# BharathMasetty/DPG-SLAM

Measured on AMD Instinct MI355X. Metric: ICP edges/sec + ms/GN-iter on 5k-node/20k-edge synthetic graph, 1->8 GPU, higher is better.
Workload: dtype fp32 (ICP) + fp64 (GN)

## Files before the change

### dpg-slam_amd/csrc/dpg_chol.h

```cpp
#ifndef DPG_CHOL_H
#define DPG_CHOL_H

#include <stdint.h>

#include <vector>

struct dpg_chol_opts {
    int32_t max_supernode_cols = 64;
    double relax_fraction = 0.3;
    int32_t order = 0;
    int32_t merge_single = 0;
    int32_t fused = 1;
    int32_t solve_stage = -1;
    int32_t solve_maxseg = -1;
    int32_t solve_dinv = 0;
    int32_t solve_inv_cols = 0;
};

struct dpg_chol_sym {
    int64_t n = 0;
    int32_t ns = 0;
    int32_t n_levels = 0;
    int32_t max_front = 0;
    double flops = 0.0;
    std::vector<int32_t> perm, pos;
    std::vector<int32_t> sn_c0;
    std::vector<int32_t> sn_of;
    std::vector<int64_t> sn_rows_ptr;
    std::vector<int32_t> sn_rows;
    std::vector<int32_t> sn_parent;
    std::vector<int32_t> sn_level;
    std::vector<int32_t> level_ptr;
    std::vector<int32_t> level_list;
    std::vector<int64_t> child_ptr;
    std::vector<int32_t> child_list;
    std::vector<int32_t> relmap;
    std::vector<int64_t> front_off;
};

int dpg_chol_symbolic(int64_t n, const int32_t* pair_lo, const int32_t* pair_hi, int64_t n_pairs,
                      const dpg_chol_opts* opts, dpg_chol_sym* S);
int dpg_chol_order(int64_t n, const int32_t* pair_lo, const int32_t* pair_hi, int64_t n_pairs,
                   std::vector<int32_t>& perm, std::vector<std::vector<int32_t>>& pat, bool md = false);
int dpg_chol_order_nd(int64_t n, const int32_t* pair_lo, const int32_t* pair_hi, int64_t n_pairs, int32_t leaf,
                      std::vector<int32_t>& perm, std::vector<std::vector<int32_t>>& pat);
int dpg_chol_order_nd_sep(int64_t n, const int32_t* pair_lo, const int32_t* pair_hi, int64_t n_pairs, int32_t leaf,
                          int32_t starts, int32_t bal, int32_t score, bool cover, std::vector<int32_t>& perm,
                          std::vector<std::vector<int32_t>>& pat, bool par = false);
int dpg_chol_sym_from_patterns(int64_t n, const std::vector<int32_t>& perm, const std::vector<std::vector<int32_t>>& pat,
                               const dpg_chol_opts* opts, dpg_chol_sym* S);
double dpg_chol_critical_path_us(const dpg_chol_sym& S);
int dpg_chol_sym_from_csr(int64_t n, const int32_t* perm, const int64_t* cp, const int32_t* prow,
                          const dpg_chol_opts* opts, dpg_chol_sym* S);

struct dpg_chol_incsym {
    int64_t n = 0, words = 0;
    std::vector<int32_t> perm, pos;
    std::vector<uint64_t> bits;
    int64_t swords = 0;
    std::vector<uint64_t> summ;
    std::vector<int32_t> parent;
    int64_t nnz = 0;
    std::vector<int64_t> cp;
    std::vector<int32_t> rows, rows_tmp;
    std::vector<std::pair<int32_t, int32_t>> added;
};
int dpg_incsym_reset(dpg_chol_incsym* I, int64_t n, const int32_t* pair_lo, const int32_t* pair_hi, int64_t n_pairs,
                     const dpg_chol_opts* opts = nullptr);
int dpg_incsym_order(int64_t n, const int32_t* pair_lo, const int32_t* pair_hi, int64_t n_pairs,
                     std::vector<int32_t>& perm, std::vector<std::vector<int32_t>>& pat,
                     const dpg_chol_opts* opts = nullptr, bool concurrent = false);
void dpg_incsym_init(dpg_chol_incsym* I, int64_t n, std::vector<int32_t>& perm, std::vector<std::vector<int32_t>>& pat);
void dpg_incsym_append(dpg_chol_incsym* I, int64_t k);
int64_t dpg_incsym_add_edge(dpg_chol_incsym* I, int32_t a, int32_t b);
int dpg_incsym_derive(dpg_chol_incsym* I, const dpg_chol_opts* opts, dpg_chol_sym* S);


int dpg_chol_create_sym(void** h, int64_t n, const int32_t* pair_lo, const int32_t* pair_hi, int64_t n_pairs,
                        dpg_chol_sym* S, const dpg_chol_opts* opts = nullptr);
int dpg_chol_create_sym_plan(void** h, int64_t n, const int32_t* pair_lo, const int32_t* pair_hi, int64_t n_pairs,
                             dpg_chol_sym* S, const dpg_chol_opts* opts = nullptr);
int dpg_chol_create_sym_upload(void** h);
int dpg_chol_plan_blocks(void** h, int64_t n, const int32_t* pos, const int32_t* perm, const int32_t* pair_lo,
                         const int32_t* pair_hi, int64_t n_pairs);
void dpg_chol_blocks_invalidate(void* h);
void dpg_chol_build_times(void* h, double out[2]);
int dpg_chol_fused(void* h);
int dpg_chol_plan_host(int64_t n, const int32_t* pair_lo, const int32_t* pair_hi, int64_t n_pairs,
                       const dpg_chol_sym* S, const dpg_chol_opts* opts, double* ms);

#endif
```

### dpg-slam_amd/csrc/dpg_chol_sym.cpp

```cpp
#include <math.h>
#include <stdint.h>
#include <stdio.h>
#include <stdlib.h>
#include <string.h>
#include <time.h>

#include <algorithm>
#include <atomic>
#include <functional>
#include <future>
#include <memory>
#include <queue>
#include <vector>

#include "dpg_chol.h"
#include "dpg_chol_plan.h"

namespace {

void min_degree(int64_t n, const std::vector<int64_t>& aptr, const std::vector<int32_t>& adj,
                std::vector<int32_t>& perm, std::vector<std::vector<int32_t>>& pattern) {
    const int64_t W = (n + 63) / 64;
    std::vector<uint64_t> bits((size_t)(n * W), 0ull);
    std::vector<int32_t> wlo((size_t)n, (int32_t)W), whi((size_t)n, 0);
    for (int64_t v = 0; v < n; ++v)
        for (int64_t q = aptr[v]; q < aptr[v + 1]; ++q) {
            const int32_t u = adj[(size_t)q];
            bits[(size_t)(v * W + u / 64)] |= 1ull << (u % 64);
            wlo[(size_t)v] = std::min(wlo[(size_t)v], u / 64);
            whi[(size_t)v] = std::max(whi[(size_t)v], u / 64 + 1);
        }
    std::vector<int32_t> deg((size_t)n);
    for (int64_t v = 0; v < n; ++v) deg[(size_t)v] = (int32_t)(aptr[v + 1] - aptr[v]);
    std::vector<char> done((size_t)n, 0);
    perm.assign((size_t)n, -1);
    pattern.assign((size_t)n, {});
    std::vector<int32_t> nb;
    nb.reserve(1024);
    std::priority_queue<std::pair<int32_t, int32_t>, std::vector<std::pair<int32_t, int32_t>>,
                        std::greater<std::pair<int32_t, int32_t>>> heap;
    for (int64_t v = 0; v < n; ++v) heap.emplace(deg[(size_t)v], (int32_t)v);
    for (int64_t p = 0; p < n; ++p) {
        int32_t v = -1;
        while (!heap.empty()) {
            const auto top = heap.top();
            heap.pop();
            if (!done[(size_t)top.second] && top.first == deg[(size_t)top.second]) { v = top.second; break; }
        }
        done[(size_t)v] = 1;
        perm[(size_t)p] = v;
        nb.clear();
        uint64_t* bv = &bits[(size_t)(v * W)];
        const int32_t vlo = wlo[(size_t)v], vhi = whi[(size_t)v];
        for (int64_t w = vlo; w < vhi; ++w) {
            uint64_t b = bv[w];
            while (b) {
                const int t = __builtin_ctzll(b);
                b &= b - 1;
                nb.push_back((int32_t)(w * 64 + t));
            }
        }
        pattern[(size_t)p] = nb;
        for (int32_t u : nb) {
            uint64_t* bu = &bits[(size_t)(u * W)];
            for (int64_t w = vlo; w < vhi; ++w) bu[w] |= bv[w];
            bu[u / 64] &= ~(1ull << (u % 64));
            bu[v / 64] &= ~(1ull << (v % 64));
            int32_t lo = std::min(wlo[(size_t)u], vlo), hi = std::max(whi[(size_t)u], vhi);
            while (lo < hi && bu[lo] == 0) ++lo;
            while (hi > lo && bu[hi - 1] == 0) --hi;
            wlo[(size_t)u] = lo;
            whi[(size_t)u] = hi;
            int32_t d = 0;
            for (int64_t w = lo; w < hi; ++w) d += __builtin_popcountll(bu[w]);
            if (d != deg[(size_t)u]) heap.emplace(d, u);
            deg[(size_t)u] = d;
        }
        for (int64_t w = vlo; w < vhi; ++w) bv[w] = 0;
    }
}

struct NdParams {
    int32_t starts = 0, bal = 5, score = 0;
    bool cover = false;
    bool par = false;
};
struct NdShared {
    std::vector<int32_t> stamp, lvl, aux;
    std::vector<int64_t> fptr;
    std::vector<int32_t> fcnt;
    std::atomic<int32_t> next_id{0};
};
struct NdState {
    int64_t n;
    const int64_t* aptr;
    const int32_t* adj;
    const int32_t* fadj = nullptr;
    int32_t leaf;
    NdParams prm;
    NdShared* sh;
    std::vector<int32_t> queue;
    std::vector<int32_t>* out;
};
inline int32_t stamp_of(const NdState& st, int32_t v) { return __atomic_load_n(&st.sh->stamp[(size_t)v], __ATOMIC_RELAXED); }
inline void stamp_set(NdState& st, int32_t v, int32_t id) { __atomic_store_n(&st.sh->stamp[(size_t)v], id, __ATOMIC_RELAXED); }
inline int32_t nd_new_id(NdState& st) { return st.sh->next_id.fetch_add(1, std::memory_order_relaxed) + 1; }

inline const int32_t* nbr_begin(const NdState& st, int32_t v) { return st.fadj + st.sh->fptr[(size_t)v]; }
inline const int32_t* nbr_end(const NdState& st, int32_t v) { return st.fadj + st.sh->fptr[(size_t)v] + st.sh->fcnt[(size_t)v]; }

void nd_filter(NdState& st, const std::vector<int32_t>& sub, int32_t id, std::vector<int32_t>& fadj) {
    size_t tot = 0;
    for (int32_t v : sub) tot += (size_t)(st.aptr[v + 1] - st.aptr[v]);
    fadj.clear();
    fadj.reserve(tot);
    for (int32_t v : sub) {
        st.sh->fptr[(size_t)v] = (int64_t)fadj.size();
        for (int64_t t = st.aptr[v]; t < st.aptr[v + 1]; ++t) {
            const int32_t u = st.adj[(size_t)t];
            if (stamp_of(st, u) == id) fadj.push_back(u);
        }
        st.sh->fcnt[(size_t)v] = (int32_t)((int64_t)fadj.size() - st.sh->fptr[(size_t)v]);
    }
    st.fadj = fadj.data();
}

int32_t nd_bfs_into(const NdState& st, int32_t id, int32_t src, int32_t* lvl, std::vector<int32_t>& queue) {
    (void)id;
    if (queue.size() < (size_t)st.n + 1) queue.resize((size_t)st.n + 1);
    int32_t* q = queue.data();
    size_t qh = 0, qt = 1;
    q[0] = src;
    lvl[src] = 0;
    int32_t h = 0;
    while (qh < qt) {
        const int32_t v = q[qh++];
        const int32_t lv = lvl[v];
        h = std::max(h, lv);
        for (const int32_t *p = nbr_begin(st, v), *e = nbr_end(st, v); p != e; ++p) {
            const int32_t u = *p;
            const int32_t lu = lvl[u];
            const bool fresh = lu < 0;
            lvl[u] = fresh ? lv + 1 : lu;
            q[qt] = u;
            qt += fresh;
        }
    }
    queue.resize(qt);
    return h + 1;
}
int32_t nd_bfs(NdState& st, int32_t id, int32_t src) { return nd_bfs_into(st, id, src, st.sh->lvl.data(), st.queue); }

int32_t nd_degree(const NdState& st, int32_t id, int32_t v) {
    (void)id;
    return st.sh->fcnt[(size_t)v];
}

void min_degree_small(int32_t n, uint64_t* row, int32_t* perm) {
    int32_t deg[64];
    uint64_t left = n == 64 ? ~0ull : ((1ull << n) - 1);
    for (int32_t v = 0; v < n; ++v) deg[v] = __builtin_popcountll(row[v]);
    for (int32_t p = 0; p < n; ++p) {
        int32_t v = -1;
        for (uint64_t m = left; m; m &= m - 1) {
            const int32_t u = __builtin_ctzll(m);
            if (v < 0 || deg[u] < deg[v]) v = u;
        }
        left &= ~(1ull << v);
        perm[p] = v;
        const uint64_t bv = row[v];
        for (uint64_t m = bv; m; m &= m - 1) {
            const int32_t u = __builtin_ctzll(m);
            row[u] = (row[u] | bv) & ~(1ull << u) & ~(1ull << v);
            deg[u] = __builtin_popcountll(row[u]);
        }
        row[v] = 0;
    }
}

void nd_min_degree(NdState& st, const std::vector<int32_t>& sub) {
    const int32_t id = nd_new_id(st);
    for (size_t i = 0; i < sub.size(); ++i) { stamp_set(st, sub[i], id); st.sh->lvl[(size_t)sub[i]] = (int32_t)i; }
    if (sub.size() <= 64) {
        uint64_t row[64];
        int32_t lp[64];
        const int32_t n = (int32_t)sub.size();
        for (int32_t i = 0; i < n; ++i) {
            const int32_t v = sub[(size_t)i];
            row[i] = 0;
            for (int64_t t = st.aptr[v]; t < st.aptr[v + 1]; ++t)
                if (stamp_of(st, st.adj[(size_t)t]) == id) row[i] |= 1ull << st.sh->lvl[(size_t)st.adj[(size_t)t]];
        }
        min_degree_small(n, row, lp);
        for (int32_t k = 0; k < n; ++k) st.out->push_back(sub[(size_t)lp[k]]);
        return;
    }
    std::vector<int64_t> ap(sub.size() + 1, 0);
    std::vector<int32_t> aj;
    for (size_t i = 0; i < sub.size(); ++i) {
        const int32_t v = sub[i];
        for (int64_t t = st.aptr[v]; t < st.aptr[v + 1]; ++t)
            if (stamp_of(st, st.adj[(size_t)t]) == id) aj.push_back(st.sh->lvl[(size_t)st.adj[(size_t)t]]);
        ap[i + 1] = (int64_t)aj.size();
    }
    std::vector<int32_t> lp;
    std::vector<std::vector<int32_t>> lpat;
    min_degree((int64_t)sub.size(), ap, aj, lp, lpat);
    for (int32_t l : lp) st.out->push_back(sub[(size_t)l]);
}

void nd_rec(NdState& st, std::vector<int32_t>& sub);

constexpr size_t kNdParMin = 1024;
void nd_halves(NdState& st, std::vector<int32_t>& A, std::vector<int32_t>& B, const std::vector<int32_t>& S) {
    if (st.prm.par && A.size() + B.size() >= kNdParMin) {
        std::vector<int32_t> outB;
        NdState sb;
        sb.n = st.n;
        sb.aptr = st.aptr;
        sb.adj = st.adj;
        sb.leaf = st.leaf;
        sb.prm = st.prm;
        sb.sh = st.sh;
        sb.out = &outB;
        std::future<void> fb = std::async(std::launch::async, [&sb, &B] { nd_rec(sb, B); });
        nd_rec(st, A);
        fb.get();
        st.out->insert(st.out->end(), outB.begin(), outB.end());
    } else {
        nd_rec(st, A);
        nd_rec(st, B);
    }
    for (int32_t v : S) st.out->push_back(v);
}

struct NdCut {
    int32_t bm = -1;
    bool up = false;
    double sc = 0.0;
    int64_t imb = 0;
};
constexpr size_t kNdStartsParMin = 2048;
constexpr size_t kNdStartsThreads = 4;
NdCut nd_best_cut(const NdState& st, const std::vector<int32_t>& sub, int32_t id, int32_t s0, int32_t* lvl,
                  std::vector<int32_t>& queue, int32_t have_h = 0) {
    NdCut best;
    const int64_t N = (int64_t)sub.size();
    int32_t hh = have_h;
    if (hh <= 0) {
        for (int32_t v : sub) lvl[v] = -1;
        hh = nd_bfs_into(st, id, s0, lvl, queue);
    }
    if (hh < 3) return best;
    std::vector<int64_t> cnt((size_t)hh, 0), slo((size_t)hh, 0), shi((size_t)hh, 0);
    for (int32_t v : sub) {
        const int32_t l = lvl[v];
        cnt[(size_t)l]++;
        bool up = false, dn = false;
        for (const int32_t *p = nbr_begin(st, v), *e = nbr_end(st, v); p != e; ++p) {
            const int32_t lu = lvl[*p];
            up |= lu == l + 1;
            dn |= lu == l - 1;
        }
        slo[(size_t)l] += up;
        if (l > 0) shi[(size_t)l - 1] += dn;
    }
    int64_t below = 0;
    for (int32_t l = 0; l + 1 < hh; ++l) {
        const bool up = shi[(size_t)l] < slo[(size_t)l];
        const int64_t sz = up ? shi[(size_t)l] : slo[(size_t)l];
        const int64_t a_sz = below + cnt[(size_t)l] - (up ? 0 : sz), b_sz = N - a_sz - sz;
        below += cnt[(size_t)l];
        if (l == 0 || (int64_t)st.prm.bal * a_sz < N || (int64_t)st.prm.bal * b_sz < N) continue;
        const double mn = (double)std::min(a_sz, b_sz);
        const double sc = st.prm.score == 2 ? (double)sz * sqrt((double)N / mn)
                          : st.prm.score == 1 ? (double)sz * (double)N / mn : (double)sz;
        const int64_t imb = a_sz > b_sz ? a_sz - b_sz : b_sz - a_sz;
        if (best.bm < 0 || sc < best.sc || (sc == best.sc && imb < best.imb)) {
            best.bm = l; best.up = up; best.sc = sc; best.imb = imb;
        }
    }
    return best;
}

void nd_split_multi(NdState& st, std::vector<int32_t>& sub, int32_t id, int32_t src, int32_t have_h) {
    const int64_t N = (int64_t)sub.size();
    const int T = N >= 256 ? st.prm.starts : 1;
    std::vector<int32_t> starts{src};
    int32_t h_src = have_h;
    {
        if (h_src <= 0) {
            for (int32_t v : sub) st.sh->lvl[(size_t)v] = -1;
            h_src = nd_bfs(st, id, src);
        }
        const std::vector<int32_t> order(st.queue.begin(), st.queue.end());
        for (int t = 1; t < T; ++t) starts.push_back(order[(size_t)((int64_t)t * (N - 1) / T)]);
        starts.push_back(order.back());
    }
    std::vector<NdCut> cuts(starts.size());
    const int W = st.prm.par && (size_t)N >= kNdStartsParMin ? (int)std::min<size_t>(kNdStartsThreads, starts.size()) : 1;
    size_t k_shared = 0;
    for (size_t k = 0; k < starts.size(); k += (size_t)W) {
        cuts[k] = nd_best_cut(st, sub, id, starts[k], st.sh->lvl.data(), st.queue, k == 0 ? h_src : 0);
        k_shared = k;
        if (k == 0 && W > 1) {
            break;
        }
    }
    if (W > 1) {
        auto work = [&](int w) {
            std::unique_ptr<int32_t[]> lv(new int32_t[(size_t)st.n]);
            std::vector<int32_t> q;
            for (size_t k = (size_t)w; k < starts.size(); k += (size_t)W) cuts[k] = nd_best_cut(st, sub, id, starts[k], lv.get(), q);
        };
        std::vector<std::future<void>> fs;
        for (int w = 1; w < W; ++w) fs.push_back(std::async(std::launch::async, work, w));
        for (size_t k = (size_t)W; k < starts.size(); k += (size_t)W) {
            cuts[k] = nd_best_cut(st, sub, id, starts[k], st.sh->lvl.data(), st.queue);
            k_shared = k;
        }
        for (auto& f : fs) f.get();
    }
    int32_t bsrc = -1, bm = -1;
    bool bupper = false;
    double bsc = 0.0;
    int64_t bimb = 0;
    for (size_t k = 0; k < starts.size(); ++k) {
        const NdCut& c = cuts[k];
        if (c.bm >= 0 && (bm < 0 || c.sc < bsc || (c.sc == bsc && c.imb < bimb))) {
            bsrc = starts[k]; bm = c.bm; bupper = c.up; bsc = c.sc; bimb = c.imb;
        }
    }
    if (bm < 0) { nd_min_degree(st, sub); return; }
    if (bsrc != starts[k_shared]) {
        for (int32_t v : sub) st.sh->lvl[(size_t)v] = -1;
        nd_bfs(st, id, bsrc);
    }
    auto touches = [&](int32_t v, int32_t l) {
        for (const int32_t *p = nbr_begin(st, v), *e = nbr_end(st, v); p != e; ++p)
            if (st.sh->lvl[(size_t)*p] == l) return true;
        return false;
    };
    std::vector<int32_t> A, B, S;
    if (st.prm.cover) {
        std::vector<int32_t> X, Y;
        for (int32_t v : sub) {
            const int32_t l = st.sh->lvl[(size_t)v];
            if (l == bm && touches(v, bm + 1)) { st.sh->aux[(size_t)v] = (int32_t)X.size(); X.push_back(v); }
            else if (l == bm + 1 && touches(v, bm)) { st.sh->aux[(size_t)v] = (int32_t)Y.size(); Y.push_back(v); }
        }
        std::vector<int64_t> xp(X.size() + 1, 0);
        std::vector<int32_t> xa;
        for (size_t i = 0; i < X.size(); ++i) {
            const int32_t v = X[i];
            for (const int32_t *p = nbr_begin(st, v), *e = nbr_end(st, v); p != e; ++p)
                if (st.sh->lvl[(size_t)*p] == bm + 1) xa.push_back(st.sh->aux[(size_t)*p]);
            xp[i + 1] = (int64_t)xa.size();
        }
        std::vector<int32_t> mx(X.size(), -1), my(Y.size(), -1), seen(Y.size(), -1);
        std::vector<std::pair<int32_t, int64_t>> stk;
        for (int32_t x0 = 0; x0 < (int32_t)X.size(); ++x0) {
            stk.assign(1, {x0, xp[(size_t)x0]});
            bool found = false;
            while (!stk.empty() && !found) {
                auto& top = stk.back();
                const int32_t x = top.first;
                if (top.second == xp[(size_t)x + 1]) { stk.pop_back(); continue; }
                const int32_t y = xa[(size_t)top.second++];
                if (seen[(size_t)y] == x0) continue;
                seen[(size_t)y] = x0;
                if (my[(size_t)y] < 0) {
                    int32_t yy = y;
                    for (size_t k = stk.size(); k-- > 0;) {
                        const int32_t xx = stk[k].first, prev = mx[(size_t)xx];
                        mx[(size_t)xx] = yy;
                        my[(size_t)yy] = xx;
                        yy = prev;
                    }
                    found = true;
                } else {
                    stk.push_back({my[(size_t)y], xp[(size_t)my[(size_t)y]]});
                }
            }
        }
        std::vector<char> zx(X.size(), 0), zy(Y.size(), 0);
        std::vector<int32_t> q;
        for (int32_t x = 0; x < (int32_t)X.size(); ++x)
            if (mx[(size_t)x] < 0) { zx[(size_t)x] = 1; q.push_back(x); }
        for (size_t qi = 0; qi < q.size(); ++qi) {
            const int32_t x = q[qi];
            for (int64_t t = xp[(size_t)x]; t < xp[(size_t)x + 1]; ++t) {
                const int32_t y = xa[(size_t)t];
                if (zy[(size_t)y] || mx[(size_t)x] == y) continue;
                zy[(size_t)y] = 1;
                const int32_t x2 = my[(size_t)y];
                if (x2 >= 0 && !zx[(size_t)x2]) { zx[(size_t)x2] = 1; q.push_back(x2); }
            }
        }
        for (size_t i = 0; i < X.size(); ++i) st.sh->aux[(size_t)X[i]] = zx[i] ? -1 : -2;
        for (size_t j = 0; j < Y.size(); ++j) st.sh->aux[(size_t)Y[j]] = zy[j] ? -2 : -1;
        for (int32_t v : sub) {
            const int32_t l = st.sh->lvl[(size_t)v];
            const bool in_cover = (l == bm || l == bm + 1) && st.sh->aux[(size_t)v] == -2;
            (in_cover ? S : l <= bm ? A : B).push_back(v);
        }
        for (int32_t v : X) st.sh->aux[(size_t)v] = -1;
        for (int32_t v : Y) st.sh->aux[(size_t)v] = -1;
    } else {
        for (int32_t v : sub) {
            const int32_t l = st.sh->lvl[(size_t)v];
            if (!bupper) {
                if (l < bm) A.push_back(v);
                else if (l > bm) B.push_back(v);
                else (touches(v, bm + 1) ? S : A).push_back(v);
            } else {
                if (l <= bm) A.push_back(v);
                else if (l > bm + 1) B.push_back(v);
                else (touches(v, bm) ? S : B).push_back(v);
            }
        }
    }
    nd_halves(st, A, B, S);
}

void nd_rec(NdState& st, std::vector<int32_t>& sub) {
    if ((int32_t)sub.size() <= st.leaf) { nd_min_degree(st, sub); return; }
    const int32_t id = nd_new_id(st);
    for (int32_t v : sub) { stamp_set(st, v, id); st.sh->lvl[(size_t)v] = -1; }
    std::vector<int32_t> fadj;
    nd_filter(st, sub, id, fadj);
    std::vector<std::vector<int32_t>> comps;
    int32_t comp_h = 0;
    for (int32_t v : sub)
        if (st.sh->lvl[(size_t)v] < 0) {
            comp_h = nd_bfs(st, id, v);
            comps.emplace_back(st.queue.begin(), st.queue.end());
        }
    if (comps.size() > 1) {
        for (auto& c : comps) {
            std::sort(c.begin(), c.end());
            nd_rec(st, c);
        }
        return;
    }
    int32_t src = sub[0], h = 0;
    int32_t bfs_src = -1, bfs_h = 0;
    for (int it = 0; it < 4; ++it) {
        int32_t hh = it == 0 ? comp_h : 0;
        if (hh <= 0) {
            for (int32_t v : sub) st.sh->lvl[(size_t)v] = -1;
            hh = nd_bfs(st, id, src);
        }
        bfs_src = src;
        bfs_h = hh;
        if (hh <= h) break;
        h = hh;
        int32_t best = -1, bd = 1 << 30;
        for (int32_t v : st.queue)
            if (st.sh->lvl[(size_t)v] == h - 1) {
                const int32_t d = nd_degree(st, id, v);
                if (d < bd || (d == bd && v < best)) { bd = d; best = v; }
            }
        if (best == src) break;
        src = best;
    }
    if (st.prm.starts > 0) { nd_split_multi(st, sub, id, src, bfs_src == src ? bfs_h : 0); return; }
    for (int32_t v : sub) st.sh->lvl[(size_t)v] = -1;
    h = nd_bfs(st, id, src);
    const int64_t N = (int64_t)sub.size();
    if (h < 3) { nd_min_degree(st, sub); return; }
    std::vector<int64_t> cnt((size_t)h, 0);
    for (int32_t v : sub) cnt[(size_t)st.sh->lvl[(size_t)v]]++;
    int32_t m = -1;
    int64_t below = 0, best_sz = 0, best_imb = 0;
    for (int32_t l = 0; l < h; ++l) {
        const int64_t above = N - below - cnt[(size_t)l];
        if (l > 0 && l < h - 1 && 5 * below >= N && 5 * above >= N) {
            const int64_t imb = below > above ? below - above : above - below;
            if (m < 0 || cnt[(size_t)l] < best_sz || (cnt[(size_t)l] == best_sz && imb < best_imb)) {
                m = l;
                best_sz = cnt[(size_t)l];
                best_imb = imb;
            }
        }
        below += cnt[(size_t)l];
    }
    if (m < 0) {
        below = 0;
        for (m = 0; m < h - 1 && 2 * (below + cnt[(size_t)m]) < N; ++m) below += cnt[(size_t)m];
        m = std::min(std::max(m, 1), h - 2);
    }
    auto touches = [&](int32_t v, int32_t l) {
        for (const int32_t *p = nbr_begin(st, v), *e = nbr_end(st, v); p != e; ++p)
            if (st.sh->lvl[(size_t)*p] == l) return true;
        return false;
    };
    int64_t s_lo = 0, s_hi = 0;
    for (int32_t v : sub) {
        const int32_t l = st.sh->lvl[(size_t)v];
        if (l == m) s_lo += touches(v, m + 1);
        else if (l == m + 1) s_hi += touches(v, m);
    }
    const bool upper = s_hi < s_lo;
    std::vector<int32_t> A, B, S;
    for (int32_t v : sub) {
        const int32_t l = st.sh->lvl[(size_t)v];
        if (!upper) {
            if (l < m) A.push_back(v);
            else if (l > m) B.push_back(v);
            else (touches(v, m + 1) ? S : A).push_back(v);
        } else {
            if (l <= m) A.push_back(v);
            else if (l > m + 1) B.push_back(v);
            else (touches(v, m) ? S : B).push_back(v);
        }
    }
    nd_halves(st, A, B, S);
}

void patterns_of_order(int64_t n, const std::vector<int64_t>& aptr, const std::vector<int32_t>& adj,
                       const std::vector<int32_t>& perm, std::vector<std::vector<int32_t>>& pat) {
    std::vector<int32_t> pos((size_t)n);
    for (int64_t p = 0; p < n; ++p) pos[(size_t)perm[(size_t)p]] = (int32_t)p;
    pat.assign((size_t)n, {});
    std::vector<std::vector<int32_t>> kids((size_t)n);
    std::vector<int32_t> rows, tmp;
    for (int64_t p = 0; p < n; ++p) {
        const int32_t v = perm[(size_t)p];
        rows.clear();
        for (int64_t t = aptr[v]; t < aptr[v + 1]; ++t)
            if (pos[(size_t)adj[(size_t)t]] > p) rows.push_back(pos[(size_t)adj[(size_t)t]]);
        std::sort(rows.begin(), rows.end());
        rows.erase(std::unique(rows.begin(), rows.end()), rows.end());
        for (int32_t c : kids[(size_t)p]) {
            const std::vector<int32_t>& pc = pat[(size_t)c];
            tmp.resize(rows.size() + pc.size());
            tmp.resize((size_t)(std::set_union(rows.begin(), rows.end(), pc.begin() + 1, pc.end(), tmp.begin()) - tmp.begin()));
            rows.swap(tmp);
        }
        std::vector<int32_t>().swap(kids[(size_t)p]);
        pat[(size_t)p] = rows;
        if (!rows.empty()) kids[(size_t)rows[0]].push_back((int32_t)p);
    }
}

}

int dpg_chol_order_nd(int64_t n, const int32_t* pair_lo, const int32_t* pair_hi, int64_t n_pairs, int32_t leaf,
                      std::vector<int32_t>& perm, std::vector<std::vector<int32_t>>& pat) {
    return dpg_chol_order_nd_sep(n, pair_lo, pair_hi, n_pairs, leaf, 0, 5, 0, false, perm, pat);
}

int dpg_chol_order_nd_sep(int64_t n, const int32_t* pair_lo, const int32_t* pair_hi, int64_t n_pairs, int32_t leaf,
                          int32_t starts, int32_t bal, int32_t score, bool cover, std::vector<int32_t>& perm,
                          std::vector<std::vector<int32_t>>& pat, bool par) {
    if (n <= 0) return -1;
    std::vector<int64_t> aptr((size_t)n + 1, 0);
    for (int64_t p = 0; p < n_pairs; ++p) { aptr[(size_t)pair_lo[p] + 1]++; aptr[(size_t)pair_hi[p] + 1]++; }
    for (int64_t v = 0; v < n; ++v) aptr[(size_t)v + 1] += aptr[(size_t)v];
    std::vector<int32_t> adj((size_t)aptr[(size_t)n]);
    {
        std::vector<int64_t> cur(aptr.begin(), aptr.end() - 1);
        for (int64_t p = 0; p < n_pairs; ++p) {
            adj[(size_t)cur[(size_t)pair_lo[p]]++] = pair_hi[p];
            adj[(size_t)cur[(size_t)pair_hi[p]]++] = pair_lo[p];
        }
    }
    NdState st;
    st.n = n;
    st.aptr = aptr.data();
    st.adj = adj.data();
    st.leaf = std::max<int32_t>(leaf, 4);
    st.prm.starts = starts;
    st.prm.bal = std::max<int32_t>(bal, 2);
    st.prm.score = score;
    st.prm.cover = cover && starts > 0;
    st.prm.par = par;
    NdShared sh;
    sh.aux.assign((size_t)n, -1);
    sh.stamp.assign((size_t)n, 0);
    sh.lvl.assign((size_t)n, -1);
    sh.fptr.assign((size_t)n, 0);
    sh.fcnt.assign((size_t)n, 0);
    st.sh = &sh;
    perm.clear();
    perm.reserve((size_t)n);
    st.out = &perm;
    std::vector<int32_t> all((size_t)n);
    for (int64_t v = 0; v < n; ++v) all[(size_t)v] = (int32_t)v;
    nd_rec(st, all);
    if ((int64_t)perm.size() != n) return -1;
    patterns_of_order(n, aptr, adj, perm, pat);
    return 0;
}

int dpg_chol_order(int64_t n, const int32_t* pair_lo, const int32_t* pair_hi, int64_t n_pairs,
                   std::vector<int32_t>& perm, std::vector<std::vector<int32_t>>& pat, bool md) {
    if (n <= 0) return -1;
    if (!md) return dpg_chol_order_nd(n, pair_lo, pair_hi, n_pairs, 16, perm, pat);
    std::vector<int64_t> aptr((size_t)n + 1, 0);
    for (int64_t p = 0; p < n_pairs; ++p) { aptr[(size_t)pair_lo[p] + 1]++; aptr[(size_t)pair_hi[p] + 1]++; }
    for (int64_t v = 0; v < n; ++v) aptr[(size_t)v + 1] += aptr[(size_t)v];
    std::vector<int32_t> adj((size_t)aptr[(size_t)n]);
    {
        std::vector<int64_t> cur(aptr.begin(), aptr.end() - 1);
        for (int64_t p = 0; p < n_pairs; ++p) {
            adj[(size_t)cur[(size_t)pair_lo[p]]++] = pair_hi[p];
            adj[(size_t)cur[(size_t)pair_hi[p]]++] = pair_lo[p];
        }
    }
    min_degree(n, aptr, adj, perm, pat);
    std::vector<int32_t> pos((size_t)n);
    for (int64_t p = 0; p < n; ++p) pos[(size_t)perm[(size_t)p]] = (int32_t)p;
    for (int64_t p = 0; p < n; ++p) {
        for (int32_t& u : pat[(size_t)p]) u = pos[(size_t)u];
        std::sort(pat[(size_t)p].begin(), pat[(size_t)p].end());
    }
    return 0;
}

double dpg_chol_critical_path_us(const dpg_chol_sym& S) {
    std::vector<double> cp((size_t)S.ns, 0.0);
    double crit = 0.0;
    for (int32_t s = S.ns - 1; s >= 0; --s) {
        const int32_t k = S.sn_c0[(size_t)s + 1] - S.sn_c0[(size_t)s];
        const int32_t r = (int32_t)(S.sn_rows_ptr[(size_t)s + 1] - S.sn_rows_ptr[(size_t)s]);
        const int32_t nch = (int32_t)(S.child_ptr[(size_t)s + 1] - S.child_ptr[(size_t)s]);
        const int32_t p = S.sn_parent[(size_t)s];
        cp[(size_t)s] = dpg_chol::front_est_us(3 * (k + r), 3 * k, nch) + (p >= 0 ? cp[(size_t)p] : 0.0);
        crit = std::max(crit, cp[(size_t)s]);
    }
    return crit;
}

int dpg_chol_symbolic(int64_t n, const int32_t* pair_lo, const int32_t* pair_hi, int64_t n_pairs,
                      const dpg_chol_opts* opts, dpg_chol_sym* S) {
    std::vector<int32_t> perm;
    std::vector<std::vector<int32_t>> pat;
    const int32_t order = opts ? opts->order : 0;
    if (order != 0 || n < 256) {
        if (dpg_chol_order(n, pair_lo, pair_hi, n_pairs, perm, pat, order == 1)) return -1;
        return dpg_chol_sym_from_patterns(n, perm, pat, opts, S);
    }
    struct Cand { int32_t starts, bal, score; };
    static const Cand cands[] = {{0, 5, 0}, {8, 4, 2}};
    struct Res {
        int rc = 0;
        double cp = 0.0;
        dpg_chol_sym T;
    };
    auto run = [&](int k) {
        Res r;
        std::vector<int32_t> pm;
        std::vector<std::vector<int32_t>> pt;
        if (dpg_chol_order_nd_sep(n, pair_lo, pair_hi, n_pairs, 16, cands[k].starts, cands[k].bal, cands[k].score, true,
                                  pm, pt, true) ||
            dpg_chol_sym_from_patterns(n, pm, pt, opts, &r.T))
            r.rc = -1;
        else
            r.cp = dpg_chol_critical_path_us(r.T);
        return r;
    };
    std::future<Res> second = std::async(std::launch::async, run, 1);
    Res r0 = run(0);
    Res r1 = second.get();
    if (r0.rc || r1.rc) return -1;
    *S = std::move(r1.cp < r0.cp ? r1.T : r0.T);
    return 0;
}

int dpg_chol_sym_from_patterns(int64_t n, const std::vector<int32_t>& perm, const std::vector<std::vector<int32_t>>& pat,
                               const dpg_chol_opts* opts, dpg_chol_sym* S) {
    if (n <= 0 || (int64_t)perm.size() != n || (int64_t)pat.size() != n) return -1;
    std::vector<int64_t> cp((size_t)n + 1, 0);
    for (int64_t p = 0; p < n; ++p) cp[(size_t)p + 1] = cp[(size_t)p] + (int64_t)pat[(size_t)p].size();
    std::vector<int32_t> rows((size_t)cp[(size_t)n]);
    for (int64_t p = 0; p < n; ++p) std::copy(pat[(size_t)p].begin(), pat[(size_t)p].end(), rows.begin() + cp[(size_t)p]);
    return dpg_chol_sym_from_csr(n, perm.data(), cp.data(), rows.data(), opts, S);
}

#ifdef DPG_PLAN_TIMING
double dpg_csr_t[8];
static double csr_now() {
    struct timespec ts;
    clock_gettime(CLOCK_MONOTONIC, &ts);
    return (double)ts.tv_sec * 1e3 + (double)ts.tv_nsec * 1e-6;
}
#define CSR_T(k) dpg_csr_t[k] += csr_now()
#else
#define CSR_T(k) do { } while (0)
#endif

static int sym_from_csr(int64_t n, const int32_t* perm, const int64_t* cp, const int32_t* prow, const dpg_chol_opts* opts,
                        dpg_chol_sym* S, bool exact);

int dpg_chol_sym_from_csr(int64_t n, const int32_t* perm, const int64_t* cp, const int32_t* prow,
                          const dpg_chol_opts* opts, dpg_chol_sym* S) {
    return sym_from_csr(n, perm, cp, prow, opts, S, false);
}

static int sym_from_csr(int64_t n, const int32_t* perm, const int64_t* cp, const int32_t* prow, const dpg_chol_opts* opts,
                        dpg_chol_sym* S, bool exact) {
    if (n <= 0) return -1;
    CSR_T(0);
    auto psize = [&](int64_t p) { return cp[p + 1] - cp[p]; };
    thread_local std::vector<int32_t> parent, nchild, sn_first, mark, rowbuf, stamp, mergebuf;
    parent.assign((size_t)n, -1);
    nchild.assign((size_t)n, 0);
    for (int64_t p = 0; p < n; ++p)
        if (psize(p) > 0) { parent[(size_t)p] = prow[cp[p]]; nchild[(size_t)parent[(size_t)p]]++; }
    S->sn_of.resize((size_t)n);
    sn_first.clear();
    const int32_t max_cols = opts && opts->max_supernode_cols > 0 ? opts->max_supernode_cols : 64;
    const double relax = opts ? opts->relax_fraction : 0.0;
    const bool any_child = !(opts && opts->merge_single);
    {
        int32_t s = -1;
        int64_t zeros = 0, cols = 0;
        for (int64_t p = 0; p < n; ++p) {
            bool join = false;
            if (p > 0 && s >= 0) {
                const int64_t q = p - 1;
                const int64_t cq = psize(q), cpp = psize(p);
                const int64_t ncols = p - sn_first[(size_t)s] + 1;
                const bool chain = parent[(size_t)q] == (int32_t)p &&
                                   (nchild[(size_t)p] == 1 || (any_child && ncols + cpp <= 127));
                if (chain && ncols <= max_cols) {
                    if (cq == cpp + 1) join = true;
                    else if (relax > 0.0) {
                        const int64_t add = std::max<int64_t>(0, cpp - (cq - 1)) * cols;
                        if ((double)(zeros + add) <= relax * (double)((cols + 1) * (cpp + 1))) { join = true; zeros += add; }
                    }
                }
            }
            if (!join) { sn_first.push_back((int32_t)p); ++s; zeros = 0; cols = 0; }
            S->sn_of[(size_t)p] = s;
            ++cols;
        }
    }
    const int32_t ns = (int32_t)sn_first.size();
    sn_first.push_back((int32_t)n);
    CSR_T(1);
    S->n = n;
    S->ns = ns;
    S->perm.assign(perm, perm + n);
    S->pos.resize((size_t)n);
    for (int64_t p = 0; p < n; ++p) S->pos[(size_t)perm[p]] = (int32_t)p;
    S->sn_c0.assign(sn_first.begin(), sn_first.end());
    S->sn_rows_ptr.assign((size_t)ns + 1, 0);
    S->sn_rows.clear();
    S->sn_parent.assign((size_t)ns, -1);
    mark.assign((size_t)n, -1);
    for (int32_t s = 0; s < ns; ++s) {
        const int32_t c0 = sn_first[(size_t)s], c1 = sn_first[(size_t)s + 1];
#ifndef DPG_PLAN_VERIFY
        if (exact) {
            const int32_t *b = prow + cp[c1 - 1], *e = prow + cp[c1];
            S->sn_rows.insert(S->sn_rows.end(), b, e);
            S->sn_rows_ptr[(size_t)s + 1] = (int64_t)S->sn_rows.size();
            if (e > b) S->sn_parent[(size_t)s] = S->sn_of[(size_t)*b];
            continue;
        }
#endif
        rowbuf.assign(prow + cp[c1 - 1], prow + cp[c1]);
        for (int32_t c = c1 - 2; c >= c0; --c) {
            const int32_t* b = std::lower_bound(prow + cp[c], prow + cp[c + 1], c1);
            const int32_t* e = prow + cp[c + 1];
            if (std::includes(rowbuf.begin(), rowbuf.end(), b, e)) continue;
#ifdef DPG_PLAN_VERIFY
            if (exact) {
                fprintf(stderr, "exact patterns: column %d's rows past its supernode are not in the last column's\n", c);
                abort();
            }
#endif
            mergebuf.resize(rowbuf.size() + (size_t)(e - b));
            mergebuf.resize((size_t)(std::set_union(rowbuf.begin(), rowbuf.end(), b, e, mergebuf.begin()) - mergebuf.begin()));
            rowbuf.swap(mergebuf);
        }
        S->sn_rows.insert(S->sn_rows.end(), rowbuf.begin(), rowbuf.end());
        S->sn_rows_ptr[(size_t)s + 1] = (int64_t)S->sn_rows.size();
        if (!rowbuf.empty()) S->sn_parent[(size_t)s] = S->sn_of[(size_t)rowbuf[0]];
    }
    CSR_T(2);
    S->sn_level.assign((size_t)ns, 0);
    for (int32_t s = 0; s < ns; ++s) {
        const int32_t p = S->sn_parent[(size_t)s];
        if (p >= 0) S->sn_level[(size_t)p] = std::max(S->sn_level[(size_t)p], S->sn_level[(size_t)s] + 1);
    }
    int32_t nl = 0;
    for (int32_t s = 0; s < ns; ++s) nl = std::max(nl, S->sn_level[(size_t)s] + 1);
    S->n_levels = nl;
    S->level_ptr.assign((size_t)nl + 1, 0);
    for (int32_t s = 0; s < ns; ++s) S->level_ptr[(size_t)S->sn_level[(size_t)s] + 1]++;
    for (int32_t l = 0; l < nl; ++l) S->level_ptr[(size_t)l + 1] += S->level_ptr[(size_t)l];
    S->level_list.resize((size_t)ns);
    {
        rowbuf.assign(S->level_ptr.begin(), S->level_ptr.end() - 1);
        for (int32_t s = 0; s < ns; ++s) S->level_list[(size_t)rowbuf[(size_t)S->sn_level[(size_t)s]]++] = s;
    }
    CSR_T(3);
    S->child_ptr.assign((size_t)ns + 1, 0);
    for (int32_t s = 0; s < ns; ++s)
        if (S->sn_parent[(size_t)s] >= 0) S->child_ptr[(size_t)S->sn_parent[(size_t)s] + 1]++;
    for (int32_t s = 0; s < ns; ++s) S->child_ptr[(size_t)s + 1] += S->child_ptr[(size_t)s];
    S->child_list.resize((size_t)S->child_ptr[(size_t)ns]);
    {
        rowbuf.resize((size_t)ns);
        for (int32_t s = 0; s < ns; ++s) rowbuf[(size_t)s] = (int32_t)S->child_ptr[(size_t)s];
        for (int32_t s = 0; s < ns; ++s)
            if (S->sn_parent[(size_t)s] >= 0) S->child_list[(size_t)rowbuf[(size_t)S->sn_parent[(size_t)s]]++] = s;
    }
    S->relmap.resize(S->sn_rows.size());
    stamp.assign((size_t)n, -1);
    for (int32_t p = 0; p < ns; ++p) {
        if (S->child_ptr[(size_t)p + 1] == S->child_ptr[(size_t)p]) continue;
        const int32_t pc0 = sn_first[(size_t)p], pk = sn_first[(size_t)p + 1] - pc0;
        for (int32_t c = 0; c < pk; ++c) { mark[(size_t)(pc0 + c)] = c; stamp[(size_t)(pc0 + c)] = p; }
        for (int64_t t = S->sn_rows_ptr[(size_t)p]; t < S->sn_rows_ptr[(size_t)p + 1]; ++t) {
            mark[(size_t)S->sn_rows[(size_t)t]] = pk + (int32_t)(t - S->sn_rows_ptr[(size_t)p]);
            stamp[(size_t)S->sn_rows[(size_t)t]] = p;
        }
        for (int64_t ci = S->child_ptr[(size_t)p]; ci < S->child_ptr[(size_t)p + 1]; ++ci) {
            const int32_t s = S->child_list[(size_t)ci];
            for (int64_t t = S->sn_rows_ptr[(size_t)s]; t < S->sn_rows_ptr[(size_t)s + 1]; ++t) {
                const int32_t row = S->sn_rows[(size_t)t];
                if (stamp[(size_t)row] != p) return -2;
                S->relmap[(size_t)t] = mark[(size_t)row];
            }
        }
    }
    CSR_T(4);
    S->front_off.assign((size_t)ns + 1, 0);
    double flops = 0.0;
    int32_t maxm = 0;
    for (int32_t s = 0; s < ns; ++s) {
        const int64_t k = sn_first[(size_t)s + 1] - sn_first[(size_t)s];
        const int64_t r = S->sn_rows_ptr[(size_t)s + 1] - S->sn_rows_ptr[(size_t)s];
        const int64_t m3 = 3 * (k + r);
        S->front_off[(size_t)s + 1] = S->front_off[(size_t)s] + ((m3 * m3 + 1) & ~(int64_t)1);
        maxm = std::max<int32_t>(maxm, (int32_t)(k + r));
        const double k3 = 3.0 * (double)k, r3 = 3.0 * (double)r;
        flops += k3 * k3 * k3 / 3.0 + k3 * k3 * r3 + k3 * r3 * r3;
    }
    S->max_front = maxm;
    S->flops = flops;
    CSR_T(5);
    return 0;
}

namespace {

void incsym_grow_words(dpg_chol_incsym* I, int64_t need_bits) {
    if (need_bits <= I->words * 64) return;
    int64_t w = std::max<int64_t>(64, I->words * 2);
    while (w * 64 < need_bits) w *= 2;
    const int64_t sw = (w + 63) / 64;
    std::vector<uint64_t> nb((size_t)(I->n * w), 0ull), ns((size_t)(I->n * sw), 0ull);
    for (int64_t p = 0; p < I->n; ++p) {
        memcpy(&nb[(size_t)(p * w)], &I->bits[(size_t)(p * I->words)], sizeof(uint64_t) * (size_t)I->words);
        memcpy(&ns[(size_t)(p * sw)], &I->summ[(size_t)(p * I->swords)], sizeof(uint64_t) * (size_t)I->swords);
    }
    I->bits.swap(nb);
    I->summ.swap(ns);
    I->words = w;
    I->swords = sw;
}

inline bool has(const dpg_chol_incsym* I, int64_t j, int64_t r) {
    return (I->bits[(size_t)(j * I->words + r / 64)] >> (r % 64)) & 1ull;
}

inline void set_bit(dpg_chol_incsym* I, int64_t j, int64_t r) {
    const int64_t w = r / 64;
    I->bits[(size_t)(j * I->words + w)] |= 1ull << (r % 64);
    I->summ[(size_t)(j * I->swords + w / 64)] |= 1ull << (w % 64);
}

template <typename F>
inline void for_rows_after(const dpg_chol_incsym* I, int64_t j, int64_t after, F&& f) {
    const uint64_t* row = &I->bits[(size_t)(j * I->words)];
    const uint64_t* sm = &I->summ[(size_t)(j * I->swords)];
    const int64_t w0 = (after + 1) / 64;
    for (int64_t sw = w0 / 64; sw < I->swords; ++sw) {
        uint64_t s = sm[sw];
        if (sw == w0 / 64) s &= ~0ull << (w0 % 64);
        while (s) {
            const int64_t w = sw * 64 + __builtin_ctzll(s);
            s &= s - 1;
            uint64_t m = row[w];
            if (w == w0) m &= ~0ull << ((after + 1) % 64);
            while (m) {
                f(w * 64 + __builtin_ctzll(m));
                m &= m - 1;
            }
        }
    }
}

}

int dpg_incsym_order(int64_t n, const int32_t* pair_lo, const int32_t* pair_hi, int64_t n_pairs,
                     std::vector<int32_t>& perm, std::vector<std::vector<int32_t>>& pat,
                     const dpg_chol_opts* opts, bool concurrent) {
    const int32_t order = opts ? opts->order : 0;
    int rc = 0;
    if (order == 0 && n >= 256) {
        const dpg_chol_opts o = opts ? *opts : dpg_chol_opts{};
        struct Cand {
            int rc = 0;
            double cp = 0.0;
            std::vector<int32_t> pm;
            std::vector<std::vector<int32_t>> pt;
        };
        auto run = [&](int k) {
            Cand c;
            c.rc = k == 0 ? dpg_chol_order_nd_sep(n, pair_lo, pair_hi, n_pairs, 16, 0, 5, 0, false, c.pm, c.pt, concurrent)
                          : dpg_chol_order_nd_sep(n, pair_lo, pair_hi, n_pairs, 16, 8, 4, 2, true, c.pm, c.pt, concurrent);
            if (c.rc == 0) {
                dpg_chol_sym T;
                if (dpg_chol_sym_from_patterns(n, c.pm, c.pt, &o, &T)) c.rc = -1;
                else c.cp = dpg_chol_critical_path_us(T);
            }
            return c;
        };
        std::future<Cand> second = std::async(concurrent ? std::launch::async : std::launch::deferred, run, 1);
        Cand c0 = run(0);
        Cand c1 = second.get();
        if (c0.rc || c1.rc) return -1;
        Cand& b = c1.cp < c0.cp ? c1 : c0;
        perm.swap(b.pm);
        pat.swap(b.pt);
    } else {
        rc = dpg_chol_order(n, pair_lo, pair_hi, n_pairs, perm, pat, order == 1);
    }
    return rc ? -1 : 0;
}

int dpg_incsym_reset(dpg_chol_incsym* I, int64_t n, const int32_t* pair_lo, const int32_t* pair_hi, int64_t n_pairs,
                     const dpg_chol_opts* opts) {
    std::vector<int32_t> perm;
    std::vector<std::vector<int32_t>> pat;
    if (dpg_incsym_order(n, pair_lo, pair_hi, n_pairs, perm, pat, opts, true)) return -1;
    dpg_incsym_init(I, n, perm, pat);
    return 0;
}

void dpg_incsym_init(dpg_chol_incsym* I, int64_t n, std::vector<int32_t>& perm, std::vector<std::vector<int32_t>>& pat) {
    I->n = n;
    I->words = std::max<int64_t>(64, (n + 63) / 64 * 2);
    I->swords = (I->words + 63) / 64;
    I->perm.swap(perm);
    I->pos.assign((size_t)n, 0);
    const std::vector<int32_t>& pm = I->perm;
    for (int64_t p = 0; p < n; ++p) I->pos[(size_t)pm[(size_t)p]] = (int32_t)p;
    I->bits.assign((size_t)(n * I->words), 0ull);
    I->summ.assign((size_t)(n * I->swords), 0ull);
    I->parent.assign((size_t)n, -1);
    I->nnz = 0;
    I->cp.assign((size_t)n + 1, 0);
    I->rows.clear();
    I->added.clear();
    for (int64_t p = 0; p < n; ++p) {
        for (int32_t r : pat[(size_t)p]) set_bit(I, p, r);
        I->rows.insert(I->rows.end(), pat[(size_t)p].begin(), pat[(size_t)p].end());
        I->cp[(size_t)p + 1] = (int64_t)I->rows.size();
        if (!pat[(size_t)p].empty()) I->parent[(size_t)p] = pat[(size_t)p][0];
        I->nnz += (int64_t)pat[(size_t)p].size();
    }
}

void dpg_incsym_append(dpg_chol_incsym* I, int64_t k) {
    if (k <= 0) return;
    incsym_grow_words(I, I->n + k);
    for (int64_t q = 0; q < k; ++q) {
        I->perm.push_back((int32_t)(I->n + q));
        I->pos.push_back((int32_t)(I->n + q));
        I->parent.push_back(-1);
    }
    I->n += k;
    I->bits.resize((size_t)(I->n * I->words), 0ull);
    I->summ.resize((size_t)(I->n * I->swords), 0ull);
    I->cp.resize((size_t)I->n + 1, I->cp.empty() ? 0 : I->cp.back());
}

int64_t dpg_incsym_add_edge(dpg_chol_incsym* I, int32_t a, int32_t b) {
    int64_t pa = I->pos[(size_t)a], pb = I->pos[(size_t)b];
    if (pa == pb) return 0;
    if (pa > pb) std::swap(pa, pb);
    int64_t added = 0;
    std::vector<std::pair<int64_t, int64_t>> work{{pa, pb}};
    while (!work.empty()) {
        int64_t j = work.back().first;
        const int64_t r = work.back().second;
        work.pop_back();
        while (j >= 0 && j < r) {
            if (has(I, j, r)) break;
            set_bit(I, j, r);
            I->added.emplace_back((int32_t)j, (int32_t)r);
            ++added;
            const int64_t p_old = I->parent[(size_t)j];
            if (p_old < 0 || r < p_old) {
                I->parent[(size_t)j] = (int32_t)r;
                for_rows_after(I, j, r, [&](int64_t t) { work.emplace_back(r, t); });
                break;
            }
            j = p_old;
        }
    }
    I->nnz += added;
    return added;
}

int dpg_incsym_derive(dpg_chol_incsym* I, const dpg_chol_opts* opts, dpg_chol_sym* S) {
    const int64_t n = I->n;
    if ((int64_t)I->cp.size() != n + 1) return -3;
    if (!I->added.empty()) {
        std::sort(I->added.begin(), I->added.end());
        std::vector<int32_t>& out = I->rows_tmp;
        out.resize(I->rows.size() + I->added.size());
        size_t a = 0, o = 0;
        int64_t prev = 0;
        for (int64_t p = 0; p < n; ++p) {
            const int64_t b = prev, e = I->cp[(size_t)p + 1];
            prev = e;
            I->cp[(size_t)p] = (int64_t)o;
            if (a == I->added.size() || I->added[a].first != p) {
                if (e > b) memcpy(out.data() + o, I->rows.data() + b, sizeof(int32_t) * (size_t)(e - b));
                o += (size_t)(e - b);
                continue;
            }
            int64_t t = b;
            while (a < I->added.size() && I->added[a].first == p) {
                const int32_t r = I->added[a++].second;
                while (t < e && I->rows[(size_t)t] < r) out[o++] = I->rows[(size_t)t++];
                out[o++] = r;
            }
            while (t < e) out[o++] = I->rows[(size_t)t++];
        }
        I->cp[(size_t)n] = (int64_t)o;
        out.resize(o);
        I->rows.swap(out);
        I->added.clear();
    }
    if (I->cp[(size_t)n] != I->nnz) return -3;
    return sym_from_csr(n, I->perm.data(), I->cp.data(), I->rows.data(), opts, S, true);
}
```

Measured before the change: 2.488 million.

## Add FM-style vertex separator refinement as a third nested-dissection ordering candidate

Adds a Fiduciary-Mattheyses style vertex-separator refinement pass that moves separator vertices to either side when that lowers the separator score, rolling each pass back to its best prefix. A third ordering candidate (multi-start, refined separators) is computed in parallel with the existing two, and the candidate with the lowest estimated critical path is kept. The aim is smaller separators and therefore cheaper supernodal Cholesky fronts in the GN solve, at the cost of extra host-side symbolic-analysis time and one more thread.

```diff
diff --git a/dpg-slam_amd/csrc/dpg_chol.h b/dpg-slam_amd/csrc/dpg_chol.h
--- a/dpg-slam_amd/csrc/dpg_chol.h
+++ b/dpg-slam_amd/csrc/dpg_chol.h
@@ -46,7 +46,9 @@
                       std::vector<int32_t>& perm, std::vector<std::vector<int32_t>>& pat);
 int dpg_chol_order_nd_sep(int64_t n, const int32_t* pair_lo, const int32_t* pair_hi, int64_t n_pairs, int32_t leaf,
                           int32_t starts, int32_t bal, int32_t score, bool cover, std::vector<int32_t>& perm,
-                          std::vector<std::vector<int32_t>>& pat, bool par = false);
+                          std::vector<std::vector<int32_t>>& pat, bool par = false, int32_t refine = 0);
+int dpg_chol_nd_refine(int64_t n, const int32_t* pair_lo, const int32_t* pair_hi, int64_t n_pairs, int32_t bal,
+                       int32_t score, int32_t refine, std::vector<int32_t>& side);
 int dpg_chol_sym_from_patterns(int64_t n, const std::vector<int32_t>& perm, const std::vector<std::vector<int32_t>>& pat,
                                const dpg_chol_opts* opts, dpg_chol_sym* S);
 double dpg_chol_critical_path_us(const dpg_chol_sym& S);
diff --git a/dpg-slam_amd/csrc/dpg_chol_sym.cpp b/dpg-slam_amd/csrc/dpg_chol_sym.cpp
--- a/dpg-slam_amd/csrc/dpg_chol_sym.cpp
+++ b/dpg-slam_amd/csrc/dpg_chol_sym.cpp
@@ -84,6 +84,7 @@
     int32_t starts = 0, bal = 5, score = 0;
     bool cover = false;
     bool par = false;
+    int32_t refine = 0;
 };
 struct NdShared {
     std::vector<int32_t> stamp, lvl, aux;
@@ -281,6 +282,142 @@
         }
     }
     return best;
+}
+
+constexpr int64_t kNdRefineMin = 256;
+void nd_refine(NdState& st, const std::vector<int32_t>& sub, std::vector<int32_t>& A, std::vector<int32_t>& B,
+               std::vector<int32_t>& S) {
+    const int64_t N = (int64_t)sub.size();
+    if (A.empty() || B.empty() || S.empty()) return;
+    int32_t* pos = st.sh->aux.data();
+    for (int64_t i = 0; i < N; ++i) pos[sub[(size_t)i]] = (int32_t)i;
+    enum : uint8_t { kA = 0, kB = 1, kS = 2 };
+    std::vector<uint8_t> side((size_t)N, kS);
+    for (int32_t v : A) side[(size_t)pos[v]] = kA;
+    for (int32_t v : B) side[(size_t)pos[v]] = kB;
+    int64_t sz[3] = {(int64_t)A.size(), (int64_t)B.size(), (int64_t)S.size()};
+    const int64_t bal = st.prm.bal;
+    auto score_of = [&](int64_t s, int64_t a, int64_t b) {
+        const double mn = (double)std::min(a, b);
+        if (mn <= 0.0) return HUGE_VAL;
+        return st.prm.score == 2 ? (double)s * sqrt((double)N / mn)
+               : st.prm.score == 1 ? (double)s * (double)N / mn : (double)s;
+    };
+    std::vector<int32_t> cnt[2];
+    cnt[0].resize((size_t)N);
+    cnt[1].resize((size_t)N);
+    std::vector<char> locked((size_t)N, 0), mark((size_t)N, 0);
+    std::vector<int32_t> sep, sep0;
+    std::vector<std::pair<int32_t, uint8_t>> log;
+    auto count = [&](int32_t i) {
+        int32_t c[3] = {0, 0, 0};
+        const int32_t v = sub[(size_t)i];
+        for (const int32_t *p = nbr_begin(st, v), *e = nbr_end(st, v); p != e; ++p) c[side[(size_t)pos[*p]]]++;
+        cnt[0][(size_t)i] = c[kA];
+        cnt[1][(size_t)i] = c[kB];
+    };
+    auto set_side = [&](int32_t i, uint8_t to) {
+        const uint8_t from = side[(size_t)i];
+        log.emplace_back(i, from);
+        side[(size_t)i] = to;
+        sz[from]--;
+        sz[to]++;
+        const int32_t v = sub[(size_t)i];
+        for (const int32_t *p = nbr_begin(st, v), *e = nbr_end(st, v); p != e; ++p) {
+            const int32_t j = pos[*p];
+            if (side[(size_t)j] != kS) continue;
+            if (from != kS) cnt[from][(size_t)j]--;
+            if (to != kS) cnt[to][(size_t)j]++;
+        }
+        if (to == kS) count(i);
+    };
+    for (int32_t v : S) sep.push_back(pos[v]);
+    const int32_t limit = (int32_t)std::min<int64_t>(100, std::max<int64_t>(15, N / 100));
+    bool changed = false;
+    for (int32_t pass = 0; pass < st.prm.refine; ++pass) {
+        for (int32_t i : sep) count(i);
+        sep0 = sep;
+        log.clear();
+        double best_sc = score_of(sz[kS], sz[kA], sz[kB]);
+        int64_t best_imb = sz[kA] > sz[kB] ? sz[kA] - sz[kB] : sz[kB] - sz[kA];
+        size_t best_len = 0;
+        for (int32_t bad = 0; bad < limit;) {
+            int32_t bi = -1, bto = 0, bgain = 0;
+            size_t bk = 0;
+            for (size_t k = 0; k < sep.size(); ++k) {
+                const int32_t i = sep[k];
+                if (locked[(size_t)i]) continue;
+                for (int32_t to = 0; to < 2; ++to) {
+                    const int32_t other = 1 - to, pulled = cnt[other][(size_t)i];
+                    if (pulled > 0 && bal * (sz[other] - pulled) < N) continue;
+                    const int32_t gain = 1 - pulled;
+                    bool better = bi < 0 || gain > bgain;
+                    if (!better && gain == bgain) {
+                        const bool small = sz[to] < sz[other], bsmall = sz[bto] < sz[1 - bto];
+                        better = small != bsmall ? small : i < bi;
+                    }
+                    if (better) { bi = i; bto = to; bgain = gain; bk = k; }
+                }
+            }
+            if (bi < 0) break;
+            sep[bk] = sep.back();
+            sep.pop_back();
+            locked[(size_t)bi] = 1;
+            set_side(bi, (uint8_t)bto);
+            const int32_t v = sub[(size_t)bi];
+            for (const int32_t *p = nbr_begin(st, v), *e = nbr_end(st, v); p != e; ++p) {
+                const int32_t j = pos[*p];
+                if (side[(size_t)j] == 1 - bto) { set_side(j, kS); sep.push_back(j); }
+            }
+            const double sc = score_of(sz[kS], sz[kA], sz[kB]);
+            const int64_t imb = sz[kA] > sz[kB] ? sz[kA] - sz[kB] : sz[kB] - sz[kA];
+            if (sc < best_sc || (sc == best_sc && imb < best_imb)) {
+                best_sc = sc;
+                best_imb = imb;
+                best_len = log.size();
+                bad = 0;
+            } else {
+                ++bad;
+            }
+        }
+        for (size_t k = log.size(); k-- > best_len;) {
+            const int32_t i = log[k].first;
+            sz[side[(size_t)i]]--;
+            side[(size_t)i] = log[k].second;
+            sz[side[(size_t)i]]++;
+        }
+        sep.clear();
+        auto take = [&](int32_t i) {
+            locked[(size_t)i] = 0;
+            if (side[(size_t)i] == kS && !mark[(size_t)i]) { mark[(size_t)i] = 1; sep.push_back(i); }
+        };
+        for (int32_t i : sep0) take(i);
+        for (auto& m : log) take(m.first);
+        for (int32_t i : sep) mark[(size_t)i] = 0;
+        if (best_len == 0) break;
+        changed = true;
+    }
+    if (changed) {
+        A.clear();
+        B.clear();
+        S.clear();
+        for (int64_t i = 0; i < N; ++i) (side[(size_t)i] == kA ? A : side[(size_t)i] == kB ? B : S).push_back(sub[(size_t)i]);
+    }
+#ifdef DPG_ND_VERIFY
+    for (int64_t i = 0; i < N; ++i) {
+        const int32_t v = sub[(size_t)i];
+        for (const int32_t *p = nbr_begin(st, v), *e = nbr_end(st, v); p != e; ++p)
+            if (side[(size_t)i] != kS && side[(size_t)pos[*p]] != kS && side[(size_t)pos[*p]] != side[(size_t)i]) {
+                fprintf(stderr, "nd_refine: edge %d - %d joins the two sides\n", v, *p);
+                abort();
+            }
+    }
+    if ((int64_t)(A.size() + B.size() + S.size()) != N || A.empty() || B.empty()) {
+        fprintf(stderr, "nd_refine: sides %zu + %zu + %zu of %lld\n", A.size(), B.size(), S.size(), (long long)N);
+        abort();
+    }
+#endif
+    for (int32_t v : sub) pos[v] = -1;
 }
 
 void nd_split_multi(NdState& st, std::vector<int32_t>& sub, int32_t id, int32_t src, int32_t have_h) {
@@ -420,6 +557,7 @@
             }
         }
     }
+    if (st.prm.refine > 0 && N >= kNdRefineMin) nd_refine(st, sub, A, B, S);
     nd_halves(st, A, B, S);
 }
 
@@ -553,7 +691,7 @@
 
 int dpg_chol_order_nd_sep(int64_t n, const int32_t* pair_lo, const int32_t* pair_hi, int64_t n_pairs, int32_t leaf,
                           int32_t starts, int32_t bal, int32_t score, bool cover, std::vector<int32_t>& perm,
-                          std::vector<std::vector<int32_t>>& pat, bool par) {
+                          std::vector<std::vector<int32_t>>& pat, bool par, int32_t refine) {
     if (n <= 0) return -1;
     std::vector<int64_t> aptr((size_t)n + 1, 0);
     for (int64_t p = 0; p < n_pairs; ++p) { aptr[(size_t)pair_lo[p] + 1]++; aptr[(size_t)pair_hi[p] + 1]++; }
@@ -576,6 +714,7 @@
     st.prm.score = score;
     st.prm.cover = cover && starts > 0;
     st.prm.par = par;
+    st.prm.refine = starts > 0 ? std::max<int32_t>(refine, 0) : 0;
     NdShared sh;
     sh.aux.assign((size_t)n, -1);
     sh.stamp.assign((size_t)n, 0);
@@ -594,6 +733,48 @@
     return 0;
 }
 
+int dpg_chol_nd_refine(int64_t n, const int32_t* pair_lo, const int32_t* pair_hi, int64_t n_pairs, int32_t bal,
+                       int32_t score, int32_t refine, std::vector<int32_t>& side) {
+    if (n <= 0 || (int64_t)side.size() != n) return -1;
+    std::vector<int64_t> aptr((size_t)n + 1, 0);
+    for (int64_t p = 0; p < n_pairs; ++p) { aptr[(size_t)pair_lo[p] + 1]++; aptr[(size_t)pair_hi[p] + 1]++; }
+    for (int64_t v = 0; v < n; ++v) aptr[(size_t)v + 1] += aptr[(size_t)v];
+    std::vector<int32_t> adj((size_t)aptr[(size_t)n]);
+    {
+        std::vector<int64_t> cur(aptr.begin(), aptr.end() - 1);
+        for (int64_t p = 0; p < n_pairs; ++p) {
+            adj[(size_t)cur[(size_t)pair_lo[p]]++] = pair_hi[p];
+            adj[(size_t)cur[(size_t)pair_hi[p]]++] = pair_lo[p];
+        }
+    }
+    NdState st;
+    st.n = n;
+    st.aptr = aptr.data();
+    st.adj = adj.data();
+    st.leaf = 16;
+    st.prm.bal = std::max<int32_t>(bal, 2);
+    st.prm.score = score;
+    st.prm.refine = std::max<int32_t>(refine, 0);
+    NdShared sh;
+    sh.aux.assign((size_t)n, -1);
+    sh.stamp.assign((size_t)n, 1);
+    sh.fptr.assign((size_t)n, 0);
+    sh.fcnt.assign((size_t)n, 0);
+    st.sh = &sh;
+    std::vector<int32_t> sub((size_t)n), A, B, S, fadj;
+    for (int64_t v = 0; v < n; ++v) {
+        sub[(size_t)v] = (int32_t)v;
+        if (side[(size_t)v] < 0 || side[(size_t)v] > 2) return -1;
+        (side[(size_t)v] == 0 ? A : side[(size_t)v] == 1 ? B : S).push_back((int32_t)v);
+    }
+    nd_filter(st, sub, 1, fadj);
+    if (st.prm.refine > 0) nd_refine(st, sub, A, B, S);
+    for (int32_t v : A) side[(size_t)v] = 0;
+    for (int32_t v : B) side[(size_t)v] = 1;
+    for (int32_t v : S) side[(size_t)v] = 2;
+    return 0;
+}
+
 int dpg_chol_order(int64_t n, const int32_t* pair_lo, const int32_t* pair_hi, int64_t n_pairs,
                    std::vector<int32_t>& perm, std::vector<std::vector<int32_t>>& pat, bool md) {
     if (n <= 0) return -1;
@@ -633,6 +814,7 @@
     return crit;
 }
 
+constexpr int32_t kNdRefinePasses = 4;
 int dpg_chol_symbolic(int64_t n, const int32_t* pair_lo, const int32_t* pair_hi, int64_t n_pairs,
                       const dpg_chol_opts* opts, dpg_chol_sym* S) {
     std::vector<int32_t> perm;
@@ -642,8 +824,9 @@
         if (dpg_chol_order(n, pair_lo, pair_hi, n_pairs, perm, pat, order == 1)) return -1;
         return dpg_chol_sym_from_patterns(n, perm, pat, opts, S);
     }
-    struct Cand { int32_t starts, bal, score; };
-    static const Cand cands[] = {{0, 5, 0}, {8, 4, 2}};
+    struct Cand { int32_t starts, bal, score, refine; };
+    static const Cand cands[] = {{0, 5, 0, 0}, {8, 4, 2, 0}, {8, 4, 0, kNdRefinePasses}};
+    constexpr int kCands = (int)(sizeof(cands) / sizeof(cands[0]));
     struct Res {
         int rc = 0;
         double cp = 0.0;
@@ -654,18 +837,24 @@
         std::vector<int32_t> pm;
         std::vector<std::vector<int32_t>> pt;
         if (dpg_chol_order_nd_sep(n, pair_lo, pair_hi, n_pairs, 16, cands[k].starts, cands[k].bal, cands[k].score, true,
-                                  pm, pt, true) ||
+                                  pm, pt, true, cands[k].refine) ||
             dpg_chol_sym_from_patterns(n, pm, pt, opts, &r.T))
             r.rc = -1;
         else
             r.cp = dpg_chol_critical_path_us(r.T);
         return r;
     };
-    std::future<Res> second = std::async(std::launch::async, run, 1);
-    Res r0 = run(0);
-    Res r1 = second.get();
-    if (r0.rc || r1.rc) return -1;
-    *S = std::move(r1.cp < r0.cp ? r1.T : r0.T);
+    std::future<Res> later[kCands - 1];
+    for (int k = 1; k < kCands; ++k) later[k - 1] = std::async(std::launch::async, run, k);
+    Res res[kCands];
+    res[0] = run(0);
+    for (int k = 1; k < kCands; ++k) res[k] = later[k - 1].get();
+    int b = 0;
+    for (int k = 0; k < kCands; ++k) {
+        if (res[k].rc) return -1;
+        if (res[k].cp < res[b].cp) b = k;
+    }
+    *S = std::move(res[b].T);
     return 0;
 }
 
```

Result: faster. 2.547 million, median of 6 (+2.4%).
